# Ssellu/vslam-pose-estimation-framework

Hardware: AMD Instinct MI355X
Metric: stereo frames/sec on KITTI-00 at 1/2/4/8 MI355X; ATE vs reference (higher is better)
Workload: dtype u8

## Files before the change

vslam_pose_estimation_framework_amd/csrc/kernels_image.h:

```cpp
#pragma once
#include <hip/hip_runtime.h>
#include "dev_types.h"
#include "../../include/vslam_brief_pattern.h"
#include "../../include/vslam_orb_pattern.h"
#include "brief_footprint.h"

__constant__ int8_t c_brief[256][4] = VSLAM_BRIEF_PATTERN_INIT;
constexpr int8_t k_brief_builtin[256][4] = VSLAM_BRIEF_PATTERN_INIT;
constexpr BriefFootprint k_brief_builtin_fp = brief_footprint(k_brief_builtin);
__constant__ BriefFootprint c_brief_fp = k_brief_builtin_fp;
__constant__ int8_t c_orb[256][4] = VSLAM_ORB_PATTERN_INIT;

__device__ __forceinline__ size_t ix_side(const DevCfg& c, int s, int d) { return (size_t)s * 2 + d; }
__device__ __forceinline__ uint16_t* box_of(const DevCfg& c, const DevBuf& b, int s, int d) {
  return b.box + ix_side(c, s, d) * (size_t)c.c.rows * c.bstride;
}
__device__ __forceinline__ uint8_t* score_of(const DevCfg& c, const DevBuf& b, int s, int d) {
  return b.score8 + ix_side(c, s, d) * (size_t)c.c.rows * c.bstride;
}
__device__ __forceinline__ unsigned long long* mask_of(const DevCfg& c, const DevBuf& b, int s, int d) {
  return b.mask + ix_side(c, s, d) * (size_t)c.c.rows * c.TX;
}
__device__ __forceinline__ int16_t* kpxy_of(const DevCfg& c, const DevBuf& b, int s, int d) {
  return b.kp_xy + ix_side(c, s, d) * (size_t)c.NMAX * 2;
}
__device__ __forceinline__ uint8_t* kpscore_of(const DevCfg& c, const DevBuf& b, int s, int d) {
  return b.kp_score + ix_side(c, s, d) * (size_t)c.NMAX;
}
__device__ __forceinline__ uint8_t* desc_of(const DevCfg& c, const DevBuf& b, int s, int d) {
  return b.desc + ix_side(c, s, d) * (size_t)c.NMAX * 32;
}
__device__ __forceinline__ int32_t* rowcell_of(const DevCfg& c, const DevBuf& b, int s, int d) {
  return b.rowcell + ix_side(c, s, d) * (size_t)c.c.rows * (c.CW + 1);
}
__device__ __forceinline__ uint8_t* used_of(const DevCfg& c, const DevBuf& b, int s, int d) {
  return b.used + ix_side(c, s, d) * (size_t)c.NMAX;
}
__device__ __forceinline__ int32_t* kill_of(const DevCfg& c, const DevBuf& b, int s, int d) {
  return b.kill + ix_side(c, s, d) * (size_t)c.NMAX;
}

__device__ __forceinline__ int block_exclusive_scan(int v, int* sh, int* total) {
  const int lane = threadIdx.x & 63, w = threadIdx.x >> 6, nw = blockDim.x >> 6;
  int inc = v;
#pragma unroll
  for (int o = 1; o < 64; o <<= 1) {
    const int t = __shfl_up(inc, o, 64);
    if (lane >= o) inc += t;
  }
  __syncthreads();
  if (lane == 63) sh[w] = inc;
  __syncthreads();
  if (threadIdx.x == 0) {
    int acc = 0;
    for (int i = 0; i < nw; ++i) { const int t = sh[i]; sh[i] = acc; acc += t; }
    sh[16] = acc;
  }
  __syncthreads();
  *total = sh[16];
  return sh[w] + inc - v;
}

__device__ __forceinline__ void xcd_tile(int* tx, int* ty, int* tz, int mono = 0, int rot = 0) {
  const int gx = gridDim.x, gy = gridDim.y;
  const int tps = mono ? gx * gy : gx * gy * 2;
  const int ns = mono ? gridDim.z : gridDim.z >> 1;
  int lin = blockIdx.x + gx * (blockIdx.y + gy * blockIdx.z);
  const int per = (ns >> 3) * tps;
  if (lin < (per << 3)) { const int x = (lin + rot) & 7, j = lin >> 3, q = j / tps; lin = (x + 8 * q) * tps + (j - q * tps); }
  *tx = lin % gx;
  const int r = lin / gx;
  *ty = r % gy;
  *tz = r / gy;
}

__device__ __forceinline__ int region_threshold(const DevCfg& c, const int32_t* thr, int x, int y) {
  for (int r = 0; r < c.n_regions; ++r) {
    const DevRegion& R = c.regions[r];
    if (x >= R.x + 3 && x < R.x + R.w - 3 && y >= R.y + 3 && y < R.y + R.h - 3) return thr[r];
  }
  return -1;
}

typedef short s16x2 __attribute__((ext_vector_type(2)));
__device__ __forceinline__ s16x2 pk_min(s16x2 a, s16x2 b) { return __builtin_elementwise_min(a, b); }
__device__ __forceinline__ s16x2 pk_max(s16x2 a, s16x2 b) { return __builtin_elementwise_max(a, b); }

__device__ __forceinline__ void fast_pair_scores(const uint8_t (*t)[80], int ly0, int lx0, int ly1, int lx1, int thr0, int thr1,
                                                 int* s0, int* s1) {
  const int dx[16] = {0, 1, 2, 3, 3, 3, 2, 1, 0, -1, -2, -3, -3, -3, -2, -1};
  const int dy[16] = {3, 3, 2, 1, 0, -1, -2, -3, -3, -3, -2, -1, 0, 1, 2, 3};
  const s16x2 v = {(short)t[ly0][lx0], (short)t[ly1][lx1]};
  s16x2 d[16];
#pragma unroll
  for (int k = 0; k < 16; ++k) {
    const s16x2 p = {(short)t[ly0 + dy[k]][lx0 + dx[k]], (short)t[ly1 + dy[k]][lx1 + dx[k]]};
    d[k] = v - p;
  }
  s16x2 mn2[16], mx2[16], mn4[16], mx4[16];
#pragma unroll
  for (int k = 0; k < 16; ++k) { mn2[k] = pk_min(d[k], d[(k + 1) & 15]); mx2[k] = pk_max(d[k], d[(k + 1) & 15]); }
#pragma unroll
  for (int k = 0; k < 16; ++k) { mn4[k] = pk_min(mn2[k], mn2[(k + 2) & 15]); mx4[k] = pk_max(mx2[k], mx2[(k + 2) & 15]); }
  s16x2 A = {-1000, -1000}, Bm = {1000, 1000};
#pragma unroll
  for (int k = 0; k < 16; ++k) {
    A = pk_max(A, pk_min(pk_min(mn4[k], mn4[(k + 4) & 15]), d[(k + 8) & 15]));
    Bm = pk_min(Bm, pk_max(pk_max(mx4[k], mx4[(k + 4) & 15]), d[(k + 8) & 15]));
  }
  const int a0 = A.x, b0 = -Bm.x, a1 = A.y, b1 = -Bm.y;
  *s0 = (thr0 >= 0 && (a0 > thr0 || b0 > thr0)) ? max(thr0, max(a0, b0)) - 1 : 0;
  *s1 = (thr1 >= 0 && (a1 > thr1 || b1 > thr1)) ? max(thr1, max(a1, b1)) - 1 : 0;
}

#define VS_FB_QCAP ((VS_TILE_H + 2) * 66)
#define VS_FB_HS_BYTES ((VS_TILE_H + 8) * VS_TILE_W * 2)
#define VS_FB_DYN_LDS (((VS_FB_QCAP + 256) * 2) > VS_FB_HS_BYTES ? ((VS_FB_QCAP + 256) * 2) : VS_FB_HS_BYTES)
__global__ __launch_bounds__(256, 8) void k_fast_box(const DevCfg c, const DevBuf b) {
  extern __shared__ __align__(16) unsigned char fb_dyn[];
  __shared__ __align__(16) uint8_t tile[VS_TILE_H + 8][80];
  __shared__ __align__(4) uint8_t sc[VS_TILE_H + 2][68];
  __shared__ int32_t s_thr[VSLAM_MAX_REGIONS];
  constexpr int QCAP = VS_FB_QCAP;
  uint16_t* queue = reinterpret_cast<uint16_t*>(fb_dyn);
  uint16_t (*hs)[VS_TILE_W] = reinterpret_cast<uint16_t (*)[VS_TILE_W]>(fb_dyn);
  __shared__ unsigned long long lmask[VS_TILE_H];
  __shared__ int qn;
  int tx, ty, tz;
  xcd_tile(&tx, &ty, &tz, c.mono, b.xcd_rot);
  const int s = b.s0 + (c.mono ? tz : (tz >> 1)), side = c.mono ? 0 : (tz & 1);
  if (!vs_active(b, s)) return;
  const int x0 = tx * VS_TILE_W, y0 = ty * VS_TILE_H;
  const int rows = c.c.rows, cols = c.c.cols;
  const uint8_t* img = b.img[side] + (size_t)s * b.img_stream_stride;
  const int stride = b.img_row_stride;
  const int tid = threadIdx.x, lane = tid & 63, w = tid >> 6;
  if (tid < c.n_regions) s_thr[tid] = min(max(b.st[s].thr[tid], 0), 255);
  if (tid == 0) qn = 0;
  if (tid < VS_TILE_H) lmask[tid] = 0ull;
  for (int i = tid; i < (VS_TILE_H + 2) * 17; i += 256) reinterpret_cast<uint32_t*>(&sc[0][0])[i] = 0u;
  const bool aligned = ((stride & 3) == 0) && ((reinterpret_cast<uintptr_t>(img) & 3) == 0);
  constexpr int NST = ((VS_TILE_H + 8) * 18 + 255) / 256;
  if (aligned && x0 >= 4 && x0 + 68 <= cols) {
    uint32_t v[NST];
#pragma unroll
    for (int u = 0; u < NST; ++u) {
      const int i = tid + 256 * u;
      const int r = i / 18, q = i - r * 18;
      const int gy = min(max(y0 - 4 + r, 0), rows - 1);
      v[u] = 0;
      if (i < (VS_TILE_H + 8) * 18) v[u] = __builtin_nontemporal_load(reinterpret_cast<const uint32_t*>(img + (size_t)gy * stride + (x0 - 4 + 4 * q)));
    }
#pragma unroll
    for (int u = 0; u < NST; ++u) {
      const int i = tid + 256 * u;
      const int r = i / 18, q = i - r * 18;
      if (i < (VS_TILE_H + 8) * 18) *reinterpret_cast<uint32_t*>(&tile[r][4 * q]) = v[u];
    }
  } else {
    for (int i = tid; i < (VS_TILE_H + 8) * 18; i += 256) {
      const int r = i / 18, q = i - r * 18;
      const int gy = min(max(y0 - 4 + r, 0), rows - 1), gx0 = x0 - 4 + 4 * q;
      uint32_t v = 0;
#pragma unroll
      for (int k = 0; k < 4; ++k) v |= (uint32_t)img[(size_t)gy * stride + min(max(gx0 + k, 0), cols - 1)] << (8 * k);
      *reinterpret_cast<uint32_t*>(&tile[r][4 * q]) = v;
    }
  }
  __syncthreads();
  int uni_thr = -2, vx0 = 0, vx1 = 0, vy0 = 0, vy1 = 0;
  bool uni_full = false;
  {
    int hits = 0;
    for (int r = 0; r < c.n_regions; ++r) {
      const DevRegion& R = c.regions[r];
      const int ax0 = max(R.x + 3, x0 - 1), ax1 = min(R.x + R.w - 3, x0 + 65), ay0 = max(R.y + 3, y0 - 1), ay1 = min(R.y + R.h - 3, y0 + VS_TILE_H + 1);
      if (ax0 < ax1 && ay0 < ay1) {
        if (hits == 0) { uni_thr = s_thr[r]; vx0 = ax0 - (x0 - 1); vx1 = ax1 - (x0 - 1); vy0 = ay0 - (y0 - 1); vy1 = ay1 - (y0 - 1); }
        ++hits;
      }
    }
    if (hits != 1) uni_thr = -2;
    uni_full = uni_thr != -2 && vx0 == 0 && vx1 == 66 && vy0 == 0 && vy1 == VS_TILE_H + 2;
  }
  auto pretest = [&](int r, int cc, bool valid = true) {
    const int thr = !valid ? -1 : (uni_full ? uni_thr : region_threshold(c, s_thr, x0 - 1 + cc, y0 - 1 + r));
    bool cand = false;
    if (thr >= 0) {
      const int ly = r + 3, lx = cc + 3;
      const int v = tile[ly][lx];
      const int d0 = v - tile[ly + 3][lx], d4 = v - tile[ly][lx + 3], d8 = v - tile[ly - 3][lx], d12 = v - tile[ly][lx - 3];
      const int dk = min(max(d0, d8), max(d4, d12));
      const int br = max(min(d0, d8), min(d4, d12));
      cand = dk > thr || br < -thr;
    }
    const unsigned long long m = __ballot(cand);
    if (m) {
      int base = 0;
      if (lane == 0) base = atomicAdd(&qn, __popcll(m));
      base = __builtin_amdgcn_readfirstlane(base);
      if (cand) queue[base + __builtin_amdgcn_mbcnt_hi((uint32_t)(m >> 32), __builtin_amdgcn_mbcnt_lo((uint32_t)m, 0u))] = (uint16_t)((r << 8) | cc);
    }
  };
  if (uni_thr != -2) {
    const s16x2 thr2 = {(short)uni_thr, (short)uni_thr};
    constexpr bool RING = (VS_TILE_H % 16) == 0;
    constexpr int RBASE = RING ? 1 : 0, RCOUNT = RING ? VS_TILE_H : VS_TILE_H + 2;
#pragma unroll 1
    for (int pass = 0; pass < (RCOUNT + 15) / 16; ++pass) {
      if (pass * 16 + w * 4 >= RCOUNT) continue;
      const int r = RBASE + pass * 16 + (tid >> 4), q = (tid & 15) + 1;
      uint32_t ng0 = 0, ng1 = 0;
      if (r < RBASE + RCOUNT) {
        const uint32_t* rowp = reinterpret_cast<const uint32_t*>(&tile[r + 3][0]);
        const uint32_t C = rowp[q], C0 = rowp[q - 1], C2 = rowp[q + 1];
        const uint32_t N = reinterpret_cast<const uint32_t*>(&tile[r][0])[q], S = reinterpret_cast<const uint32_t*>(&tile[r + 6][0])[q];
#pragma unroll
        for (int half = 0; half < 2; ++half) {
          const uint32_t sel = half ? 0x0c030c02u : 0x0c010c00u;
          const uint32_t vv = __builtin_amdgcn_perm(0u, C, sel), nn = __builtin_amdgcn_perm(0u, N, sel), ss = __builtin_amdgcn_perm(0u, S, sel);
          const uint32_t ee = __builtin_amdgcn_perm(C2, C, half ? 0x0c060c05u : 0x0c040c03u);
          const uint32_t ww = __builtin_amdgcn_perm(C, C0, half ? 0x0c040c03u : 0x0c020c01u);
          const s16x2 v = __builtin_bit_cast(s16x2, vv), n = __builtin_bit_cast(s16x2, nn), s_ = __builtin_bit_cast(s16x2, ss);
          const s16x2 e = __builtin_bit_cast(s16x2, ee), w_ = __builtin_bit_cast(s16x2, ww);
          const s16x2 lo = pk_max(pk_min(n, s_), pk_min(e, w_)), hi = pk_min(pk_max(n, s_), pk_max(e, w_));
          const uint32_t neg = __builtin_bit_cast(uint32_t, (s16x2)(lo - (v - thr2))) | __builtin_bit_cast(uint32_t, (s16x2)((v + thr2) - hi));
          if (half) ng1 = neg; else ng0 = neg;
        }
      }
      bool p0 = (short)(ng0 & 0xffffu) < 0, p1 = (int)ng0 < 0, p2 = (short)(ng1 & 0xffffu) < 0, p3 = (int)ng1 < 0;
      if (!uni_full) {
        const bool rok = r >= vy0 && r < vy1;
        const int c0 = 4 * q - 3;
        p0 = p0 && rok && c0 >= vx0 && c0 < vx1;         p1 = p1 && rok && c0 + 1 >= vx0 && c0 + 1 < vx1;
        p2 = p2 && rok && c0 + 2 >= vx0 && c0 + 2 < vx1; p3 = p3 && rok && c0 + 3 >= vx0 && c0 + 3 < vx1;
      }
      const unsigned long long m0 = __ballot(p0), m1 = __ballot(p1), m2 = __ballot(p2), m3 = __ballot(p3);
      const int n0 = __popcll(m0), n1 = __popcll(m1), n2 = __popcll(m2), n3 = __popcll(m3);
      if (n0 + n1 + n2 + n3) {
        int base = 0;
        if (lane == 0) base = atomicAdd(&qn, n0 + n1 + n2 + n3);
        base = __builtin_amdgcn_readfirstlane(base);
        const int ent = (r << 8) | (4 * q - 3);
        auto below = [&](unsigned long long m) { return (int)__builtin_amdgcn_mbcnt_hi((uint32_t)(m >> 32), __builtin_amdgcn_mbcnt_lo((uint32_t)m, 0u)); };
        const int trash = QCAP + tid;
        queue[p0 ? base + below(m0) : trash] = (uint16_t)ent;
        queue[p1 ? base + n0 + below(m1) : trash] = (uint16_t)(ent + 1);
        queue[p2 ? base + n0 + n1 + below(m2) : trash] = (uint16_t)(ent + 2);
        queue[p3 ? base + n0 + n1 + n2 + below(m3) : trash] = (uint16_t)(ent + 3);
      }
    }
    if (RING) {
      constexpr int NRING = 2 * 66 + 2 * VS_TILE_H;
      for (int i0 = 0; i0 < NRING; i0 += 256) {
        const int i = i0 + tid;
        int r = 0, cc = 0;
        if (i < 66) { r = 0; cc = i; }
        else if (i < 132) { r = VS_TILE_H + 1; cc = i - 66; }
        else { const int k = i - 132; r = 1 + (k >> 1); cc = (k & 1) ? 65 : 0; }
        pretest(r, cc, i < NRING);
      }
    } else {
      if (tid >= 64 && tid < 64 + (VS_TILE_H + 2) * 2) { const int i = tid - 64; pretest(i >> 1, (i & 1) ? 65 : 0); }
    }
  } else {
    for (int r = w; r < VS_TILE_H + 2; r += 4) pretest(r, lane);
    if (tid < (VS_TILE_H + 2) * 2) pretest(tid >> 1, 64 + (tid & 1));
    static_assert((VS_TILE_H + 2) * 2 <= 256, "one pass over the halo columns");
  }
  __syncthreads();
  {
    const int nq = qn;
    for (int q = tid; 2 * q < nq; q += 256) {
      const int e0 = queue[2 * q], e1 = (2 * q + 1 < nq) ? queue[2 * q + 1] : e0;
      const int r0 = e0 >> 8, c0 = e0 & 255, r1 = e1 >> 8, c1 = e1 & 255;
      int sv0, sv1;
      const int t0 = uni_thr != -2 ? uni_thr : region_threshold(c, s_thr, x0 - 1 + c0, y0 - 1 + r0);
      const int t1 = uni_thr != -2 ? uni_thr : region_threshold(c, s_thr, x0 - 1 + c1, y0 - 1 + r1);
      fast_pair_scores(tile, r0 + 3, c0 + 3, r1 + 3, c1 + 3, t0, t1, &sv0, &sv1);
      sc[r0][c0] = (uint8_t)sv0;
      if (2 * q + 1 < nq) sc[r1][c1] = (uint8_t)sv1;
    }
  }
  __syncthreads();
  unsigned long long* mask = mask_of(c, b, s, side);
  uint8_t* score8 = score_of(c, b, s, side);
  uint16_t* box = box_of(c, b, s, side);
  {
    const int nq = qn;
    for (int q = tid; q < nq; q += 256) {
      const int e0 = queue[q];
      const int r = e0 >> 8, cc = e0 & 255;
      if (r < 1 || r > VS_TILE_H || cc < 1 || cc > 64) continue;
      const int v = sc[r][cc];
      if (v == 0) continue;
      const bool keep = v > sc[r - 1][cc - 1] && v > sc[r - 1][cc] && v > sc[r - 1][cc + 1] && v > sc[r][cc - 1] &&
                        v > sc[r][cc + 1] && v > sc[r + 1][cc - 1] && v > sc[r + 1][cc] && v > sc[r + 1][cc + 1];
      if (keep) {
        atomicOr(&lmask[r - 1], 1ull << (cc - 1));
        const int gy = y0 + r - 1;
        if (gy < rows) score8[(size_t)gy * c.bstride + (x0 + cc - 1)] = (uint8_t)v;
      }
    }
  }
  __syncthreads();
  const bool want_box = c.c.descriptor_type == VSLAM_DESCRIPTOR_BRIEF;
  if (want_box)
  for (int i = tid; i < (VS_TILE_H + 8) * 16; i += 256) {
    const int r = i >> 4, q = i & 15;
    const uint32_t* p = reinterpret_cast<const uint32_t*>(&tile[r][4 * q]);
    const uint32_t w0 = p[0], w1 = p[1], w2 = p[2];
    const uint32_t s0 = __builtin_amdgcn_sad_u8(w0, 0u, __builtin_amdgcn_sad_u8(w1, 0u, w2 & 255u));
    const uint32_t s1 = s0 - (w0 & 255u) + ((w2 >> 8) & 255u);
    const uint32_t s2 = s1 - ((w0 >> 8) & 255u) + ((w2 >> 16) & 255u);
    const uint32_t s3 = s2 - ((w0 >> 16) & 255u) + (w2 >> 24);
    *reinterpret_cast<uint2*>(&hs[r][4 * q]) = make_uint2(s0 | (s1 << 16), s2 | (s3 << 16));
  }
  __syncthreads();
  if (want_box) {
    constexpr int RW = VS_TILE_H / 8;
    const int half = lane >> 5, px = 2 * (lane & 31);
    const int rbase = (w * 2 + half) * RW;
    typedef unsigned short u16x2 __attribute__((ext_vector_type(2)));
    u16x2 acc = {0, 0};
#pragma unroll
    for (int k = 0; k < 9; ++k) acc += *reinterpret_cast<const u16x2*>(&hs[rbase + k][px]);
#pragma unroll
    for (int j = 0; j < RW; ++j) {
      const int r = rbase + j, gy = y0 + r;
      if (gy < rows && x0 + px < c.bstride) __builtin_nontemporal_store(__builtin_bit_cast(uint32_t, acc), reinterpret_cast<uint32_t*>(box + (size_t)gy * c.bstride + x0 + px));
      if (j < RW - 1) acc += *reinterpret_cast<const u16x2*>(&hs[r + 9][px]) - *reinterpret_cast<const u16x2*>(&hs[r][px]);
    }
  }
  __syncthreads();
  if (tid < VS_TILE_H && y0 + tid < rows) mask[(size_t)(y0 + tid) * c.TX + tx] = lmask[tid];
}

__device__ __forceinline__ unsigned long long col_mask(int lo, int hi, int wx0) {
  int a = max(lo - wx0, 0), e = min(hi - wx0, 64);
  if (e <= a) return 0ull;
  const unsigned long long hi_m = (e >= 64) ? ~0ull : ((1ull << e) - 1ull);
  return hi_m & ~((1ull << a) - 1ull);
}

#ifndef VS_EMIT_WPT
#define VS_EMIT_WPT 4
#endif
__global__ __launch_bounds__(512, VS_EMIT_WPT > 8 ? 2 : 4) void k_emit(const DevCfg c, const DevBuf b, int border, int run_controller) {
  __shared__ int sh_wave[8], sh_total;
  __shared__ int sh_cnt[VSLAM_MAX_REGIONS];
  __shared__ int sh_last;
  const int s = b.s0 + xcd_local_stream(blockIdx.x, gridDim.x, (b.xcd_rot + blockIdx.y * gridDim.x) & 7), tid = threadIdx.x;
  if (!vs_active(b, s)) return;
  const int rows = c.c.rows, cols = c.c.cols, TX = c.TX, CW = c.CW;
  StreamState& st = b.st[s];
  if (tid < VSLAM_MAX_REGIONS) sh_cnt[tid] = 0;
  __syncthreads();
  const int nwords = rows * TX;
  const int side = blockIdx.y, lane = tid & 63, w = tid >> 6;
  {
    const unsigned long long* mask = mask_of(c, b, s, side);
    const uint8_t* score8 = score_of(c, b, s, side);
    int16_t* kxy = kpxy_of(c, b, s, side);
    uint8_t* ksc = kpscore_of(c, b, s, side);
    int32_t* rowcell = rowcell_of(c, b, s, side);
    uint8_t* used = used_of(c, b, s, side);
    auto filtered = [&](unsigned long long m, int row, int t) -> unsigned long long {
      const bool row_ok = row >= border && row < rows - border;
      return row_ok ? (m & col_mask(border, cols - border, t * 64)) : 0ull;
    };
    int done = 0;
    const int q64 = 64 / TX, r64 = 64 - q64 * TX;
    for (int p0 = 0; p0 < nwords; p0 += 512 * VS_EMIT_WPT) {
      const int wbase = p0 + w * 64 * VS_EMIT_WPT + lane;
      const int row_b = wbase / TX, t_b = wbase - row_b * TX;
      unsigned long long mw[VS_EMIT_WPT];
#pragma unroll
      for (int j = 0; j < VS_EMIT_WPT; ++j) mw[j] = (wbase + 64 * j < nwords) ? mask[wbase + 64 * j] : 0ull;
      for (int r = 0; r < c.n_regions; ++r) {
        const DevRegion& R = c.regions[r];
        int n = 0, row = row_b, t = t_b;
#pragma unroll
        for (int j = 0; j < VS_EMIT_WPT; ++j) {
          if (row >= R.y + 3 && row < R.y + R.h - 3) n += __popcll(mw[j] & col_mask(R.x + 3, R.x + R.w - 3, t * 64));
          t += r64; row += q64; if (t >= TX) { t -= TX; ++row; }
        }
#pragma unroll
        for (int o = 32; o > 0; o >>= 1) n += __shfl_xor(n, o, 64);
        if (lane == 0 && n) atomicAdd(&sh_cnt[r], n);
      }
      int ex[VS_EMIT_WPT];
      int carry = 0;
      int row = row_b, t = t_b;
#pragma unroll
      for (int j = 0; j < VS_EMIT_WPT; ++j) {
        const int wd = wbase + 64 * j;
        mw[j] = wd < nwords ? filtered(mw[j], row, t) : 0ull;
        t += r64; row += q64; if (t >= TX) { t -= TX; ++row; }
        const int cnt = __popcll(mw[j]);
        int inc = cnt;
#pragma unroll
        for (int o = 1; o < 64; o <<= 1) { const int up = __shfl_up(inc, o, 64); if (lane >= o) inc += up; }
        ex[j] = carry + inc - cnt;
        carry += __shfl(inc, 63, 64);
      }
      __syncthreads();
      if (lane == 0) sh_wave[w] = carry;
      __syncthreads();
      if (tid == 0) { int acc = 0; for (int i = 0; i < 8; ++i) { const int v = sh_wave[i]; sh_wave[i] = acc; acc += v; } sh_total = acc; }
      __syncthreads();
      const int wave_off = done + sh_wave[w];
      row = row_b; t = t_b;
#pragma unroll
      for (int j = 0; j < VS_EMIT_WPT; ++j) {
        const int wd = wbase + 64 * j;
        if (wd < nwords) {
          unsigned long long f = mw[j];
          int off = wave_off + ex[j];
          int32_t* rc = rowcell + (size_t)row * (CW + 1) + t * 4;
          rc[0] = min(off, c.NMAX);
          rc[1] = min(off + __popcll(f & 0xFFFFull), c.NMAX);
          rc[2] = min(off + __popcll(f & 0xFFFFFFFFull), c.NMAX);
          rc[3] = min(off + __popcll(f & 0xFFFFFFFFFFFFull), c.NMAX);
          if (t == TX - 1) rc[4] = min(off + __popcll(f), c.NMAX);
          while (f) {
            const int bit = __ffsll((long long)f) - 1;
            f &= f - 1;
            if (off < c.NMAX) {
              *reinterpret_cast<int32_t*>(kxy + 2 * off) = (t * 64 + bit) | (row << 16);
              used[off] = 0;
            }
            ++off;
          }
        }
        t += r64; row += q64; if (t >= TX) { t -= TX; ++row; }
      }
      done += sh_total;
    }
    const int total = done;
    if (total > c.NMAX) { if (tid == 0) atomicOr(&st.error_flags, 1); }
    if (tid == 0) b.n_kp[s * 2 + side] = min(total, c.NMAX);
    __syncthreads();
    const int nk = min(total, c.NMAX);
    for (int i0 = tid; i0 < nk; i0 += 4 * 512) {
      int px[4];
      uint8_t v[4];
#pragma unroll
      for (int u = 0; u < 4; ++u) {
        const int i = i0 + 512 * u;
        px[u] = (i < nk) ? *reinterpret_cast<const int32_t*>(kxy + 2 * i) : 0;
      }
#pragma unroll
      for (int u = 0; u < 4; ++u) v[u] = (i0 + 512 * u < nk) ? score8[(size_t)(px[u] >> 16) * c.bstride + (px[u] & 0xFFFF)] : 0;
#pragma unroll
      for (int u = 0; u < 4; ++u) if (i0 + 512 * u < nk) ksc[i0 + 512 * u] = v[u];
    }
    __syncthreads();
  }
  if (tid == 0) {
    for (int r = 0; r < c.n_regions; ++r) b.iinfo[s].raw_count[side][r] = sh_cnt[r];
    __threadfence();
    const int last_ticket = (int)gridDim.y - 1;
    const int ticket = atomicAdd(&b.iinfo[s].ticket, 1);
    sh_last = ticket == last_ticket;
    if (ticket == last_ticket) { __threadfence(); b.iinfo[s].ticket = 0; }
  }
  __syncthreads();
  if (tid == 0 && sh_last) {
    const int (*cnt)[VSLAM_MAX_REGIONS] = b.iinfo[s].raw_count;
    if (run_controller) {
      const double tol = c.c.target_number_of_keypoints_tolerance, maxchg = c.c.detector_threshold_maximum_change;
      const double tmin = c.c.detector_threshold_minimum, tmax = c.c.detector_threshold_maximum;
      const double target = (double)c.target_per_detector;
      const int n_sides = run_controller == 2 ? 1 : 2;
      for (int r = 0; r < c.n_regions; ++r) {
        double acc = 0;
        for (int sd = 0; sd < n_sides; ++sd) {
          double t = (double)st.thr[r];
          const double delta = ((double)__hip_atomic_load(&cnt[sd][r], __ATOMIC_RELAXED, __HIP_MEMORY_SCOPE_AGENT) - target) / target;
          if (delta < -tol) {
            const double change = fmax(delta, -maxchg);
            t = t + fmin(change * t, -1.0);
            if (t < tmin) t = tmin;
          } else if (delta > tol) {
            const double change = fmin(delta, maxchg);
            t += fmax(change * t, 1.0);
            if (t > tmax) t = tmax;
          }
          acc += t;
        }
        st.thr[r] = (int)rint(acc / n_sides);
      }
    }
    for (int r = 0; r < c.n_regions; ++r) b.iinfo[s].thr_after[r] = st.thr[r];
  }
}

__device__ __forceinline__ void brief_wave(const uint16_t* box, int bstride, int x, int y, int lane, uint8_t* out32) {
#pragma unroll
  for (int j = 0; j < 4; ++j) {
    const int i = j * 64 + lane;
    const int a = box[(size_t)(y + c_brief[i][0]) * bstride + (x + c_brief[i][1])];
    const int bb = box[(size_t)(y + c_brief[i][2]) * bstride + (x + c_brief[i][3])];
    const unsigned long long m = __ballot(a < bb);
    if (lane == 0) {
      const unsigned long long wv = __builtin_bswap64(__brevll(m));
      reinterpret_cast<unsigned long long*>(out32)[j] = wv;
    }
  }
}

#ifndef VS_BT_W
#define VS_BT_W 128
#endif
#ifndef VS_BT_H
#define VS_BT_H 64
#endif
#define VS_BT_RW (VS_BT_W + 2 * VSLAM_BRIEF_PATCH_HALF)
#define VS_BT_RH (VS_BT_H + 2 * VSLAM_BRIEF_PATCH_HALF)
__global__ __launch_bounds__(256) void k_brief(const DevCfg c, const DevBuf b) {
  __shared__ __align__(16) uint16_t reg[VS_BT_RH * VS_BT_RW];
  __shared__ int row_lo[VS_BT_H], row_off[VS_BT_H + 1];
  int tx, ty, tz;
  xcd_tile(&tx, &ty, &tz, c.mono, b.xcd_rot);
  const int s = b.s0 + (c.mono ? tz : (tz >> 1)), side = c.mono ? 0 : (tz & 1);
  if (!vs_active(b, s)) return;
  const int x0 = tx * VS_BT_W, y0 = ty * VS_BT_H;
  const int rows = c.c.rows;
  const int tid = threadIdx.x, lane = tid & 63, w = tid >> 6;
  const int32_t* rowcell = rowcell_of(c, b, s, side);
  if (tid < VS_BT_H) {
    const int r = y0 + tid;
    int lo = 0, n = 0;
    if (r < rows) {
      const int c0 = min((VS_BT_W / 16) * tx, c.CW), c1 = min((VS_BT_W / 16) * (tx + 1), c.CW);
      lo = rowcell[(size_t)r * (c.CW + 1) + c0];
      n = rowcell[(size_t)r * (c.CW + 1) + c1] - lo;
    }
    row_lo[tid] = lo;
    int inc = n;
#pragma unroll
    for (int o = 1; o < VS_BT_H; o <<= 1) { const int t = __shfl_up(inc, o, 64); if (tid >= o) inc += t; }
    row_off[tid + 1] = inc;
    if (tid == 0) row_off[0] = 0;
  }
  __syncthreads();
  const int K = row_off[VS_BT_H];
  if (K == 0) return;
  const uint16_t* box = box_of(c, b, s, side);
  constexpr int CPR = VS_BT_RW / 8;
  constexpr int NLD = (VS_BT_RH * CPR + 255) / 256;
  uint4 stage[NLD];
#pragma unroll
  for (int u = 0; u < NLD; ++u) {
    const int i = tid + 256 * u;
    const int r = i / CPR, q = i - r * CPR;
    const int gy = min(max(y0 - VSLAM_BRIEF_PATCH_HALF + r, 0), rows - 1);
    const int gx = x0 - VSLAM_BRIEF_PATCH_HALF + 8 * q;
    stage[u] = make_uint4(0u, 0u, 0u, 0u);
    if (i < VS_BT_RH * CPR && gx >= 0 && gx + 8 <= c.bstride) stage[u] = *reinterpret_cast<const uint4*>(box + (size_t)gy * c.bstride + gx);
  }
  const int16_t* kxy = kpxy_of(c, b, s, side);
  auto lookup = [&](int k, int* base, int* idx) {
    *base = 0; *idx = -1;
    if (k < K) {
      int r = 0;
#pragma unroll
      for (int step = VS_BT_H / 2; step > 0; step >>= 1) if (row_off[r + step] <= k) r += step;
      const int id = row_lo[r] + (k - row_off[r]);
      *idx = id;
      *base = (r + VSLAM_BRIEF_PATCH_HALF) * VS_BT_RW + (kxy[2 * id] - x0 + VSLAM_BRIEF_PATCH_HALF);
    }
  };
  int my_base, my_idx;
  lookup(w + 4 * lane, &my_base, &my_idx);
  int off_a[4], off_b[4];
#pragma unroll
  for (int j = 0; j < 4; ++j) {
    const int i = j * 64 + lane;
    off_a[j] = c_brief[i][0] * VS_BT_RW + c_brief[i][1];
    off_b[j] = c_brief[i][2] * VS_BT_RW + c_brief[i][3];
  }
#pragma unroll
  for (int u = 0; u < NLD; ++u) {
    const int i = tid + 256 * u;
    if (i < VS_BT_RH * CPR) *reinterpret_cast<uint4*>(&reg[8 * i]) = stage[u];
  }
  __syncthreads();
  uint8_t* desc = desc_of(c, b, s, side);
  for (int k0 = 0; k0 < K; k0 += 256) {
    if (k0 > 0) lookup(k0 + w + 4 * lane, &my_base, &my_idx);
    const int n_here = (min(K - k0, 256) - w + 3) >> 2;
    for (int i = 0; i < n_here; ++i) {
      const int base = __builtin_amdgcn_readlane(my_base, i), idx = __builtin_amdgcn_readlane(my_idx, i);
      unsigned long long word = 0;
#pragma unroll
      for (int j = 0; j < 4; ++j) {
        const unsigned long long m = __ballot(reg[base + off_a[j]] < reg[base + off_b[j]]);
        if (lane == j) word = m;
      }
      if (lane < 4) reinterpret_cast<unsigned long long*>(desc + (size_t)32 * idx)[lane] = __builtin_bswap64(__brevll(word));
    }
  }
}

__global__ __launch_bounds__(256) void k_brief_at(const uint16_t* box, int bstride, int rows, int cols, int n,
                                                  const int16_t* xy, uint8_t* keep, uint8_t* desc) {
  const int lane = threadIdx.x & 63;
  const int wave = blockIdx.x * (blockDim.x >> 6) + (threadIdx.x >> 6);
  const int nwaves = gridDim.x * (blockDim.x >> 6);
  for (int i = wave; i < n; i += nwaves) {
    const int x = xy[2 * i], y = xy[2 * i + 1];
    const bool in = x >= VSLAM_BRIEF_BORDER && x < cols - VSLAM_BRIEF_BORDER && y >= VSLAM_BRIEF_BORDER && y < rows - VSLAM_BRIEF_BORDER;
    if (lane == 0) keep[i] = in ? 1 : 0;
    if (in) brief_wave(box, bstride, x, y, lane, desc + (size_t)32 * i);
    else if (lane < 4) reinterpret_cast<unsigned long long*>(desc + (size_t)32 * i)[lane] = 0ull;
  }
}

struct Gauss7 { int32_t k[4]; };
__device__ __forceinline__ int reflect101(int p, int n) { return p < 0 ? -p : (p >= n ? 2 * n - 2 - p : p); }
__device__ __forceinline__ uint8_t* blur_of(const DevCfg& c, const DevBuf& b, int s, int d) { return reinterpret_cast<uint8_t*>(box_of(c, b, s, d)); }

__device__ __forceinline__ void gauss7_tile(const uint8_t* img, int stride, int rows, int cols, int x0, int y0, const Gauss7& g, uint8_t* out, int ostride,
                                            uint8_t (*src)[72], uint16_t (*hs)[VS_TILE_W]) {
  const int tid = threadIdx.x;
  const bool in_dwords = ((stride & 3) == 0) && ((reinterpret_cast<uintptr_t>(img) & 3) == 0) && x0 >= 4 && x0 + 68 <= cols;
  if (in_dwords) {
    constexpr int NST = ((VS_TILE_H + 6) * 18 + 255) / 256;
    uint32_t v[NST];
#pragma unroll
    for (int u = 0; u < NST; ++u) {
      const int i = tid + 256 * u;
      const int r = i / 18, q = i - 18 * r;
      const int gy = reflect101(min(y0 - 3 + r, rows + 2), rows);
      v[u] = 0;
      if (i < (VS_TILE_H + 6) * 18) v[u] = *reinterpret_cast<const uint32_t*>(img + (size_t)gy * stride + (x0 - 4 + 4 * q));
    }
#pragma unroll
    for (int u = 0; u < NST; ++u) {
      const int i = tid + 256 * u;
      const int r = i / 18, q = i - 18 * r;
      if (i < (VS_TILE_H + 6) * 18) *reinterpret_cast<uint32_t*>(&src[r][4 * q]) = v[u];
    }
  } else {
    for (int i = tid; i < (VS_TILE_H + 6) * 70; i += 256) {
      const int r = i / 70, q = i - 70 * r;
      src[r][q + 1] = img[(size_t)reflect101(min(y0 - 3 + r, rows + 2), rows) * stride + reflect101(min(x0 - 3 + q, cols + 2), cols)];
    }
  }
  __syncthreads();
  const uint32_t klo = (uint32_t)g.k[3] | ((uint32_t)g.k[2] << 8) | ((uint32_t)g.k[1] << 16) | ((uint32_t)g.k[0] << 24);
  const uint32_t khi = (uint32_t)g.k[1] | ((uint32_t)g.k[2] << 8) | ((uint32_t)g.k[3] << 16);
  for (int i = tid; i < (VS_TILE_H + 6) * 16; i += 256) {
    const int r = i >> 4, t = i & 15;
    const uint32_t* p = reinterpret_cast<const uint32_t*>(&src[r][4 * t]);
    const uint32_t w0 = p[0], w1 = p[1], w2 = p[2];
    uint32_t o[4];
#pragma unroll
    for (int j = 0; j < 4; ++j) {
      const uint32_t lo = j == 3 ? w1 : __builtin_amdgcn_alignbyte(w1, w0, 1 + j), hi = j == 3 ? w2 : __builtin_amdgcn_alignbyte(w2, w1, 1 + j);
      o[j] = __builtin_amdgcn_udot4(lo, klo, __builtin_amdgcn_udot4(hi, khi, 0u, false), false);
    }
    *reinterpret_cast<uint2*>(&hs[r][4 * t]) = make_uint2(o[0] | (o[1] << 16), o[2] | (o[3] << 16));
  }
  __syncthreads();
  const bool out_dwords = ((ostride & 3) == 0) && ((reinterpret_cast<uintptr_t>(out) & 3) == 0);
  for (int i = tid; i < VS_TILE_H * 16; i += 256) {
    const int r = i >> 4, t = i & 15;
    if (y0 + r >= rows || x0 + 4 * t >= cols) continue;
    uint32_t acc[4] = {0, 0, 0, 0};
#pragma unroll
    for (int d = 0; d < 7; ++d) {
      const uint2 v = *reinterpret_cast<const uint2*>(&hs[r + d][4 * t]);
      const uint32_t kk = (uint32_t)g.k[d < 3 ? 3 - d : d - 3];
      acc[0] += kk * (v.x & 0xFFFFu); acc[1] += kk * (v.x >> 16); acc[2] += kk * (v.y & 0xFFFFu); acc[3] += kk * (v.y >> 16);
    }
    uint32_t px[4];
#pragma unroll
    for (int j = 0; j < 4; ++j) px[j] = min((acc[j] + (1u << 15)) >> 16, 255u);
    uint8_t* dst = out + (size_t)(y0 + r) * ostride + x0 + 4 * t;
    if (out_dwords && x0 + 4 * t + 4 <= (ostride > cols ? ostride : cols)) {
      *reinterpret_cast<uint32_t*>(dst) = px[0] | (px[1] << 8) | (px[2] << 16) | (px[3] << 24);
    } else {
#pragma unroll
      for (int j = 0; j < 4; ++j) if (x0 + 4 * t + j < cols) dst[j] = (uint8_t)px[j];
    }
  }
}
__global__ __launch_bounds__(256) void k_gauss7(const DevCfg c, const DevBuf b, const Gauss7 g) {
  __shared__ uint8_t src[VS_TILE_H + 6][72];
  __shared__ uint16_t hs[VS_TILE_H + 6][VS_TILE_W];
  int tx, ty, tz;
  xcd_tile(&tx, &ty, &tz, c.mono, b.xcd_rot);
  const int s = b.s0 + (c.mono ? tz : (tz >> 1)), side = c.mono ? 0 : (tz & 1);
  if (!vs_active(b, s)) return;
  gauss7_tile(b.img[side] + (size_t)s * b.img_stream_stride, b.img_row_stride, c.c.rows, c.c.cols, tx * VS_TILE_W, ty * VS_TILE_H, g,
              blur_of(c, b, s, side), c.bstride, src, hs);
}
__global__ __launch_bounds__(256) void k_gauss7_plain(const uint8_t* img, int stride, int rows, int cols, const Gauss7 g, uint8_t* out, int ostride) {
  __shared__ uint8_t src[VS_TILE_H + 6][72];
  __shared__ uint16_t hs[VS_TILE_H + 6][VS_TILE_W];
  gauss7_tile(img, stride, rows, cols, blockIdx.x * VS_TILE_W, blockIdx.y * VS_TILE_H, g, out, ostride, src, hs);
}

struct OrbTaps { int off[4][2]; };
__device__ __forceinline__ OrbTaps orb_taps(int lane, float a, float bsin, int stride) {
  OrbTaps t;
#pragma unroll
  for (int j = 0; j < 4; ++j) {
    const int i = j * 64 + lane;
#pragma unroll
    for (int h = 0; h < 2; ++h) {
      const float px = (float)c_orb[i][2 * h], py = (float)c_orb[i][2 * h + 1];
      const float xf = px * a - py * bsin, yf = px * bsin + py * a;
      t.off[j][h] = (int)rintf(yf) * stride + (int)rintf(xf);
    }
  }
  return t;
}
__device__ __forceinline__ void orb_wave(const uint8_t* centre, const OrbTaps& t, unsigned long long d[4]) {
  int v[4][2];
#pragma unroll
  for (int j = 0; j < 4; ++j) { v[j][0] = centre[t.off[j][0]]; v[j][1] = centre[t.off[j][1]]; }
#pragma unroll
  for (int j = 0; j < 4; ++j) d[j] = __ballot(v[j][0] < v[j][1]);
}
#define VS_OT_HALF 16
#define VS_OT_RW (VS_BT_W + 2 * VS_OT_HALF)
#define VS_OT_RH (VS_BT_H + 2 * VS_OT_HALF)
__global__ __launch_bounds__(256) void k_orb_describe(const DevCfg c, const DevBuf b, float a, float bsin) {
  __shared__ __align__(16) uint8_t reg[VS_OT_RH * VS_OT_RW];
  __shared__ int row_lo[VS_BT_H], row_off[VS_BT_H + 1];
  int tx, ty, tz;
  xcd_tile(&tx, &ty, &tz, c.mono, b.xcd_rot);
  const int s = b.s0 + (c.mono ? tz : (tz >> 1)), side = c.mono ? 0 : (tz & 1);
  if (!vs_active(b, s)) return;
  const int x0 = tx * VS_BT_W, y0 = ty * VS_BT_H;
  const int rows = c.c.rows;
  const int tid = threadIdx.x, lane = tid & 63, w = tid >> 6;
  const int32_t* rowcell = rowcell_of(c, b, s, side);
  if (tid < VS_BT_H) {
    const int r = y0 + tid;
    int lo = 0, n = 0;
    if (r < rows) {
      const int c0 = min((VS_BT_W / 16) * tx, c.CW), c1 = min((VS_BT_W / 16) * (tx + 1), c.CW);
      lo = rowcell[(size_t)r * (c.CW + 1) + c0];
      n = rowcell[(size_t)r * (c.CW + 1) + c1] - lo;
    }
    row_lo[tid] = lo;
    int inc = n;
#pragma unroll
    for (int o = 1; o < VS_BT_H; o <<= 1) { const int t = __shfl_up(inc, o, 64); if (tid >= o) inc += t; }
    row_off[tid + 1] = inc;
    if (tid == 0) row_off[0] = 0;
  }
  __syncthreads();
  const int K = row_off[VS_BT_H];
  if (K == 0) return;
  const uint8_t* blur = blur_of(c, b, s, side);
  constexpr int CPR = VS_OT_RW / 16;
  constexpr int NLD = (VS_OT_RH * CPR + 255) / 256;
  uint4 stage[NLD];
#pragma unroll
  for (int u = 0; u < NLD; ++u) {
    const int i = tid + 256 * u;
    const int r = i / CPR, q = i - r * CPR;
    const int gy = min(max(y0 - VS_OT_HALF + r, 0), rows - 1);
    const int gx = x0 - VS_OT_HALF + 16 * q;
    stage[u] = make_uint4(0u, 0u, 0u, 0u);
    if (i < VS_OT_RH * CPR && gx >= 0 && gx + 16 <= c.bstride) stage[u] = *reinterpret_cast<const uint4*>(blur + (size_t)gy * c.bstride + gx);
  }
  const int16_t* kxy = kpxy_of(c, b, s, side);
  auto lookup = [&](int k, int* base, int* idx) {
    *base = 0; *idx = -1;
    if (k < K) {
      int r = 0;
#pragma unroll
      for (int step = VS_BT_H / 2; step > 0; step >>= 1) if (row_off[r + step] <= k) r += step;
      const int id = row_lo[r] + (k - row_off[r]);
      *idx = id;
      *base = (r + VS_OT_HALF) * VS_OT_RW + (kxy[2 * id] - x0 + VS_OT_HALF);
    }
  };
  int my_base, my_idx;
  lookup(w + 4 * lane, &my_base, &my_idx);
  const OrbTaps t = orb_taps(lane, a, bsin, VS_OT_RW);
#pragma unroll
  for (int u = 0; u < NLD; ++u) {
    const int i = tid + 256 * u;
    if (i < VS_OT_RH * CPR) *reinterpret_cast<uint4*>(&reg[16 * i]) = stage[u];
  }
  __syncthreads();
  uint8_t* desc = desc_of(c, b, s, side);
  for (int k0 = 0; k0 < K; k0 += 256) {
    if (k0 > 0) lookup(k0 + w + 4 * lane, &my_base, &my_idx);
    const int n_here = (min(K - k0, 256) - w + 3) >> 2;
    for (int i = 0; i < n_here; ++i) {
      const int base = __builtin_amdgcn_readlane(my_base, i), idx = __builtin_amdgcn_readlane(my_idx, i);
      unsigned long long word = 0;
#pragma unroll
      for (int j = 0; j < 4; ++j) {
        const unsigned long long m = __ballot(reg[base + t.off[j][0]] < reg[base + t.off[j][1]]);
        if (lane == j) word = m;
      }
      if (lane < 4) reinterpret_cast<unsigned long long*>(desc + (size_t)32 * idx)[lane] = word;
    }
  }
}
__global__ __launch_bounds__(256) void k_orb_at(const uint8_t* blur, int stride, int rows, int cols, int n, const int16_t* xy, float a, float bsin,
                                                uint8_t* keep, uint8_t* desc) {
  const int lane = threadIdx.x & 63;
  const int wave = blockIdx.x * (blockDim.x >> 6) + (threadIdx.x >> 6), nwaves = gridDim.x * (blockDim.x >> 6);
  const OrbTaps t = orb_taps(lane, a, bsin, stride);
  for (int i = wave; i < n; i += nwaves) {
    const int x = xy[2 * i], y = xy[2 * i + 1];
    const bool in = x >= VSLAM_ORB_BORDER && x < cols - VSLAM_ORB_BORDER && y >= VSLAM_ORB_BORDER && y < rows - VSLAM_ORB_BORDER;
    if (lane == 0) keep[i] = in ? 1 : 0;
    unsigned long long d[4] = {0ull, 0ull, 0ull, 0ull};
    if (in) orb_wave(blur + (size_t)y * stride + x, t, d);
    const unsigned long long dv = lane == 0 ? d[0] : (lane == 1 ? d[1] : (lane == 2 ? d[2] : d[3]));
    if (lane < 4) reinterpret_cast<unsigned long long*>(desc + (size_t)32 * i)[lane] = dv;
  }
}

struct OrbLevels { const uint8_t* blur[16]; int32_t stride[16], rows[16], cols[16]; };
__global__ __launch_bounds__(256) void k_orb_at_levels(const OrbLevels L, int n, const int32_t* pos, const float* ab, uint8_t* keep, uint8_t* desc) {
  const int lane = threadIdx.x & 63;
  const int wave = blockIdx.x * (blockDim.x >> 6) + (threadIdx.x >> 6), nwaves = gridDim.x * (blockDim.x >> 6);
  for (int i = wave; i < n; i += nwaves) {
    const int lv = pos[3 * i + 2];
    unsigned long long d[4] = {0ull, 0ull, 0ull, 0ull};
    const bool in = lv >= 0;
    if (in) {
      const int stride = L.stride[lv];
      const OrbTaps t = orb_taps(lane, ab[2 * i], ab[2 * i + 1], stride);
      orb_wave(L.blur[lv] + (size_t)pos[3 * i + 1] * stride + pos[3 * i], t, d);
    }
    if (lane == 0) keep[i] = in ? 1 : 0;
    const unsigned long long dv = lane == 0 ? d[0] : (lane == 1 ? d[1] : (lane == 2 ? d[2] : d[3]));
    if (lane < 4) reinterpret_cast<unsigned long long*>(desc + (size_t)32 * i)[lane] = dv;
  }
}

enum { VS_KNN_HAMMING = 0, VS_KNN_L2 = 1, VS_KNN_L1 = 2, VS_KNN_SL2 = 3 };
#define VS_KNN_TILE 256
__device__ __forceinline__ void knn_merge(unsigned long long& b0, unsigned long long& b1, unsigned long long c0, unsigned long long c1) {
  const unsigned long long lo = b0 < c0 ? b0 : c0, hi = b0 < c0 ? c0 : b0, m = b1 < c1 ? b1 : c1;
  b0 = lo; b1 = hi < m ? hi : m;
}
template <int NORM>
__device__ __forceinline__ void knn2_body(int nq, const uint8_t* __restrict__ q, int nt, const uint8_t* __restrict__ t, int32_t* idx,
                                          float* dist, uint4 (*tile)[2], uint32_t* tnorm) {
  const int tid = threadIdx.x, sub = tid & 15, grp = tid >> 4;
  const int i = blockIdx.x * 16 + grp;
  const bool dotn = NORM == VS_KNN_L2 || NORM == VS_KNN_SL2;
  uint32_t qv[8];
  uint32_t qn = 0;
  {
    const uint4* qp = reinterpret_cast<const uint4*>(q + (size_t)32 * (i < nq ? i : nq - 1));
    const uint4 a = qp[0], c = qp[1];
    qv[0] = a.x; qv[1] = a.y; qv[2] = a.z; qv[3] = a.w; qv[4] = c.x; qv[5] = c.y; qv[6] = c.z; qv[7] = c.w;
    if (dotn) {
#pragma unroll
      for (int k = 0; k < 8; ++k) qn = __builtin_amdgcn_udot4(qv[k], qv[k], qn, false);
    }
  }
  unsigned long long b0 = ~0ull, b1 = ~0ull;
  uint4 n0 = make_uint4(0, 0, 0, 0), n1 = n0;
  if (tid < nt) { const uint4* tp = reinterpret_cast<const uint4*>(t + (size_t)32 * tid); n0 = tp[0]; n1 = tp[1]; }
  for (int j0 = 0; j0 < nt; j0 += VS_KNN_TILE) {
    __syncthreads();
    {
      const int sw = (tid >> 3) & 1;
      tile[tid][sw] = n0; tile[tid][sw ^ 1] = n1;
      if (dotn) {
        uint32_t tn = 0;
        tn = __builtin_amdgcn_udot4(n0.x, n0.x, tn, false); tn = __builtin_amdgcn_udot4(n0.y, n0.y, tn, false);
        tn = __builtin_amdgcn_udot4(n0.z, n0.z, tn, false); tn = __builtin_amdgcn_udot4(n0.w, n0.w, tn, false);
        tn = __builtin_amdgcn_udot4(n1.x, n1.x, tn, false); tn = __builtin_amdgcn_udot4(n1.y, n1.y, tn, false);
        tn = __builtin_amdgcn_udot4(n1.z, n1.z, tn, false); tn = __builtin_amdgcn_udot4(n1.w, n1.w, tn, false);
        tnorm[tid] = tn;
      }
    }
    const int jn = j0 + VS_KNN_TILE;
    if (jn + tid < nt) { const uint4* tp = reinterpret_cast<const uint4*>(t + (size_t)32 * (jn + tid)); n0 = tp[0]; n1 = tp[1]; }
    __syncthreads();
    const int cnt = min(VS_KNN_TILE, nt - j0);
    for (int r = sub; r < cnt; r += 16) {
      const int sw = (r >> 3) & 1;
      const uint4 a = tile[r][sw], c = tile[r][sw ^ 1];
      const uint32_t tv[8] = {a.x, a.y, a.z, a.w, c.x, c.y, c.z, c.w};
      uint32_t d = 0;
      if (NORM == VS_KNN_HAMMING) {
#pragma unroll
        for (int k = 0; k < 8; ++k) d += __popc(qv[k] ^ tv[k]);
      } else if (NORM == VS_KNN_L1) {
#pragma unroll
        for (int k = 0; k < 8; ++k) d = __builtin_amdgcn_sad_u8(qv[k], tv[k], d);
      } else {
        uint32_t dot = 0;
#pragma unroll
        for (int k = 0; k < 8; ++k) dot = __builtin_amdgcn_udot4(qv[k], tv[k], dot, false);
        d = qn + tnorm[r] - 2u * dot;
      }
      const unsigned long long key = ((unsigned long long)d << 32) | (unsigned)(j0 + r);
      if (key < b0) { b1 = b0; b0 = key; }
      else if (key < b1) { b1 = key; }
    }
  }
#pragma unroll
  for (int m = 1; m < 16; m <<= 1) {
    const unsigned long long c0 = __shfl_xor(b0, m, 64), c1 = __shfl_xor(b1, m, 64);
    knn_merge(b0, b1, c0, c1);
  }
  if (i < nq && sub == 0) {
    const bool h0 = b0 != ~0ull, h1 = b1 != ~0ull;
    idx[2 * i] = h0 ? (int32_t)(b0 & 0xFFFFFFFFull) : -1;
    idx[2 * i + 1] = h1 ? (int32_t)(b1 & 0xFFFFFFFFull) : -1;
    const float d0 = (float)(uint32_t)(b0 >> 32), d1 = (float)(uint32_t)(b1 >> 32);
    dist[2 * i] = h0 ? (NORM == VS_KNN_L2 ? sqrtf(d0) : d0) : 0.f;
    dist[2 * i + 1] = h1 ? (NORM == VS_KNN_L2 ? sqrtf(d1) : d1) : 0.f;
  }
}
__global__ __launch_bounds__(256) void k_knn2(int norm, int nq, const uint8_t* __restrict__ q, int nt,
                                              const uint8_t* __restrict__ t, int32_t* idx, float* dist) {
  __shared__ uint4 tile[VS_KNN_TILE][2];
  __shared__ uint32_t tnorm[VS_KNN_TILE];
  if (norm == VS_KNN_HAMMING) knn2_body<VS_KNN_HAMMING>(nq, q, nt, t, idx, dist, tile, tnorm);
  else if (norm == VS_KNN_L2) knn2_body<VS_KNN_L2>(nq, q, nt, t, idx, dist, tile, tnorm);
  else if (norm == VS_KNN_L1) knn2_body<VS_KNN_L1>(nq, q, nt, t, idx, dist, tile, tnorm);
  else knn2_body<VS_KNN_SL2>(nq, q, nt, t, idx, dist, tile, tnorm);
}
```

Before: 187,000.

## Rewrite FAST score as f16 packed min3/max3 over pixels; simplify candidate queue

The FAST corner score now works on raw pixel values packed into f16 (via the 0x6400 exponent trick) and takes windowed min/max with three-input min3/max3 ops. The centre pixel is subtracted once at the end instead of forming 16 differences first. The pretest loop precomputes column-validity masks and folds the row range into one bound check. It also uses an inline-asm LDS fetch-add, replaces trash-slot stores with predicated stores, drops the queue padding, and skips wholly idle waves on the ring pass. The goal is fewer VALU instructions and less LDS use. The risks are correctness of the windowed min/max reduction, and the asm waitcnt serialising the atomic.

Result: faster. 195,100 (median of 6 runs) (+4.3%).

```diff
diff --git a/vslam_pose_estimation_framework_amd/csrc/kernels_image.h b/vslam_pose_estimation_framework_amd/csrc/kernels_image.h
--- a/vslam_pose_estimation_framework_amd/csrc/kernels_image.h
+++ b/vslam_pose_estimation_framework_amd/csrc/kernels_image.h
@@ -86,42 +86,51 @@
 __device__ __forceinline__ s16x2 pk_min(s16x2 a, s16x2 b) { return __builtin_elementwise_min(a, b); }
 __device__ __forceinline__ s16x2 pk_max(s16x2 a, s16x2 b) { return __builtin_elementwise_max(a, b); }
 
+typedef _Float16 h16x2 __attribute__((ext_vector_type(2)));
+__device__ __forceinline__ h16x2 pk_min3(h16x2 a, h16x2 b, h16x2 c) { return __builtin_elementwise_minimum(__builtin_elementwise_minimum(a, b), c); }
+__device__ __forceinline__ h16x2 pk_max3(h16x2 a, h16x2 b, h16x2 c) { return __builtin_elementwise_maximum(__builtin_elementwise_maximum(a, b), c); }
+
 __device__ __forceinline__ void fast_pair_scores(const uint8_t (*t)[80], int ly0, int lx0, int ly1, int lx1, int thr0, int thr1,
                                                  int* s0, int* s1) {
   const int dx[16] = {0, 1, 2, 3, 3, 3, 2, 1, 0, -1, -2, -3, -3, -3, -2, -1};
   const int dy[16] = {3, 3, 2, 1, 0, -1, -2, -3, -3, -3, -2, -1, 0, 1, 2, 3};
-  const s16x2 v = {(short)t[ly0][lx0], (short)t[ly1][lx1]};
-  s16x2 d[16];
-#pragma unroll
-  for (int k = 0; k < 16; ++k) {
-    const s16x2 p = {(short)t[ly0 + dy[k]][lx0 + dx[k]], (short)t[ly1 + dy[k]][lx1 + dx[k]]};
-    d[k] = v - p;
-  }
-  s16x2 mn2[16], mx2[16], mn4[16], mx4[16];
-#pragma unroll
-  for (int k = 0; k < 16; ++k) { mn2[k] = pk_min(d[k], d[(k + 1) & 15]); mx2[k] = pk_max(d[k], d[(k + 1) & 15]); }
-#pragma unroll
-  for (int k = 0; k < 16; ++k) { mn4[k] = pk_min(mn2[k], mn2[(k + 2) & 15]); mx4[k] = pk_max(mx2[k], mx2[(k + 2) & 15]); }
-  s16x2 A = {-1000, -1000}, Bm = {1000, 1000};
-#pragma unroll
-  for (int k = 0; k < 16; ++k) {
-    A = pk_max(A, pk_min(pk_min(mn4[k], mn4[(k + 4) & 15]), d[(k + 8) & 15]));
-    Bm = pk_min(Bm, pk_max(pk_max(mx4[k], mx4[(k + 4) & 15]), d[(k + 8) & 15]));
-  }
-  const int a0 = A.x, b0 = -Bm.x, a1 = A.y, b1 = -Bm.y;
+  h16x2 p[16];
+#pragma unroll
+  for (int k = 0; k < 16; ++k)
+    p[k] = __builtin_bit_cast(h16x2, (uint32_t)t[ly0 + dy[k]][lx0 + dx[k]] | ((uint32_t)t[ly1 + dy[k]][lx1 + dx[k]] << 16) | 0x64006400u);
+  h16x2 mn3[16], mx3[16], amn[16], amx[16];
+#pragma unroll
+  for (int k = 0; k < 16; ++k) { mn3[k] = pk_min3(p[k], p[(k + 1) & 15], p[(k + 2) & 15]); mx3[k] = pk_max3(p[k], p[(k + 1) & 15], p[(k + 2) & 15]); }
+#pragma unroll
+  for (int k = 0; k < 16; ++k) { amn[k] = pk_min3(mn3[k], mn3[(k + 3) & 15], mn3[(k + 6) & 15]); amx[k] = pk_max3(mx3[k], mx3[(k + 3) & 15], mx3[(k + 6) & 15]); }
+  h16x2 M6[6], m6[6];
+#pragma unroll
+  for (int k = 0; k < 5; ++k) { M6[k] = pk_min3(amx[3 * k], amx[3 * k + 1], amx[3 * k + 2]); m6[k] = pk_max3(amn[3 * k], amn[3 * k + 1], amn[3 * k + 2]); }
+  M6[5] = amx[15]; m6[5] = amn[15];
+  const h16x2 M2 = pk_min3(pk_min3(M6[0], M6[1], M6[2]), pk_min3(M6[3], M6[4], M6[5]), M6[5]);
+  const h16x2 m2 = pk_max3(pk_max3(m6[0], m6[1], m6[2]), pk_max3(m6[3], m6[4], m6[5]), m6[5]);
+  const uint32_t Mb = __builtin_bit_cast(uint32_t, M2), mb = __builtin_bit_cast(uint32_t, m2);
+  const int v0 = t[ly0][lx0], v1 = t[ly1][lx1];
+  const int a0 = v0 - (int)(Mb & 0x3ffu), b0 = (int)(mb & 0x3ffu) - v0, a1 = v1 - (int)((Mb >> 16) & 0x3ffu), b1 = (int)((mb >> 16) & 0x3ffu) - v1;
   *s0 = (thr0 >= 0 && (a0 > thr0 || b0 > thr0)) ? max(thr0, max(a0, b0)) - 1 : 0;
   *s1 = (thr1 >= 0 && (a1 > thr1 || b1 > thr1)) ? max(thr1, max(a1, b1)) - 1 : 0;
 }
 
+__device__ __forceinline__ int lds_fetch_add(int* word, int v) {
+  const uint32_t addr = (uint32_t)reinterpret_cast<uintptr_t>((__attribute__((address_space(3))) int*)word);
+  int old;
+  asm volatile("ds_add_rtn_u32 %0, %1, %2\n\ts_waitcnt lgkmcnt(0)" : "=&v"(old) : "v"(addr), "v"(v) : "memory");
+  return old;
+}
+
 #define VS_FB_QCAP ((VS_TILE_H + 2) * 66)
 #define VS_FB_HS_BYTES ((VS_TILE_H + 8) * VS_TILE_W * 2)
-#define VS_FB_DYN_LDS (((VS_FB_QCAP + 256) * 2) > VS_FB_HS_BYTES ? ((VS_FB_QCAP + 256) * 2) : VS_FB_HS_BYTES)
+#define VS_FB_DYN_LDS ((VS_FB_QCAP * 2) > VS_FB_HS_BYTES ? (VS_FB_QCAP * 2) : VS_FB_HS_BYTES)
 __global__ __launch_bounds__(256, 8) void k_fast_box(const DevCfg c, const DevBuf b) {
   extern __shared__ __align__(16) unsigned char fb_dyn[];
   __shared__ __align__(16) uint8_t tile[VS_TILE_H + 8][80];
   __shared__ __align__(4) uint8_t sc[VS_TILE_H + 2][68];
   __shared__ int32_t s_thr[VSLAM_MAX_REGIONS];
-  constexpr int QCAP = VS_FB_QCAP;
   uint16_t* queue = reinterpret_cast<uint16_t*>(fb_dyn);
   uint16_t (*hs)[VS_TILE_W] = reinterpret_cast<uint16_t (*)[VS_TILE_W]>(fb_dyn);
   __shared__ unsigned long long lmask[VS_TILE_H];
@@ -197,7 +206,7 @@
     const unsigned long long m = __ballot(cand);
     if (m) {
       int base = 0;
-      if (lane == 0) base = atomicAdd(&qn, __popcll(m));
+      if (lane == 0) base = lds_fetch_add(&qn, __popcll(m));
       base = __builtin_amdgcn_readfirstlane(base);
       if (cand) queue[base + __builtin_amdgcn_mbcnt_hi((uint32_t)(m >> 32), __builtin_amdgcn_mbcnt_lo((uint32_t)m, 0u))] = (uint16_t)((r << 8) | cc);
     }
@@ -206,12 +215,19 @@
     const s16x2 thr2 = {(short)uni_thr, (short)uni_thr};
     constexpr bool RING = (VS_TILE_H % 16) == 0;
     constexpr int RBASE = RING ? 1 : 0, RCOUNT = RING ? VS_TILE_H : VS_TILE_H + 2;
+    const int rlo = max(RBASE, vy0), rhi = min(RBASE + RCOUNT, vy1);
+    uint32_t cm0 = 0x80008000u, cm1 = 0x80008000u;
+    if (!uni_full) {
+      const int c0 = 4 * ((tid & 15) + 1) - 3;
+      cm0 = (c0 >= vx0 && c0 < vx1 ? 0x8000u : 0u) | (c0 + 1 >= vx0 && c0 + 1 < vx1 ? 0x80000000u : 0u);
+      cm1 = (c0 + 2 >= vx0 && c0 + 2 < vx1 ? 0x8000u : 0u) | (c0 + 3 >= vx0 && c0 + 3 < vx1 ? 0x80000000u : 0u);
+    }
 #pragma unroll 1
     for (int pass = 0; pass < (RCOUNT + 15) / 16; ++pass) {
-      if (pass * 16 + w * 4 >= RCOUNT) continue;
+      if (RCOUNT % 16 != 0 && pass * 16 + w * 4 >= RCOUNT) continue;
       const int r = RBASE + pass * 16 + (tid >> 4), q = (tid & 15) + 1;
       uint32_t ng0 = 0, ng1 = 0;
-      if (r < RBASE + RCOUNT) {
+      if ((unsigned)(r - rlo) < (unsigned)(rhi - rlo)) {
         const uint32_t* rowp = reinterpret_cast<const uint32_t*>(&tile[r + 3][0]);
         const uint32_t C = rowp[q], C0 = rowp[q - 1], C2 = rowp[q + 1];
         const uint32_t N = reinterpret_cast<const uint32_t*>(&tile[r][0])[q], S = reinterpret_cast<const uint32_t*>(&tile[r + 6][0])[q];
@@ -225,34 +241,30 @@
           const s16x2 e = __builtin_bit_cast(s16x2, ee), w_ = __builtin_bit_cast(s16x2, ww);
           const s16x2 lo = pk_max(pk_min(n, s_), pk_min(e, w_)), hi = pk_min(pk_max(n, s_), pk_max(e, w_));
           const uint32_t neg = __builtin_bit_cast(uint32_t, (s16x2)(lo - (v - thr2))) | __builtin_bit_cast(uint32_t, (s16x2)((v + thr2) - hi));
-          if (half) ng1 = neg; else ng0 = neg;
+          if (half) ng1 = neg & cm1; else ng0 = neg & cm0;
         }
       }
-      bool p0 = (short)(ng0 & 0xffffu) < 0, p1 = (int)ng0 < 0, p2 = (short)(ng1 & 0xffffu) < 0, p3 = (int)ng1 < 0;
-      if (!uni_full) {
-        const bool rok = r >= vy0 && r < vy1;
-        const int c0 = 4 * q - 3;
-        p0 = p0 && rok && c0 >= vx0 && c0 < vx1;         p1 = p1 && rok && c0 + 1 >= vx0 && c0 + 1 < vx1;
-        p2 = p2 && rok && c0 + 2 >= vx0 && c0 + 2 < vx1; p3 = p3 && rok && c0 + 3 >= vx0 && c0 + 3 < vx1;
-      }
+      uint32_t lo0 = ng0 << 16, lo1 = ng1 << 16;
+      asm("" : "+v"(lo0), "+v"(lo1));
+      const bool p0 = (int)lo0 < 0, p1 = (int)ng0 < 0, p2 = (int)lo1 < 0, p3 = (int)ng1 < 0;
       const unsigned long long m0 = __ballot(p0), m1 = __ballot(p1), m2 = __ballot(p2), m3 = __ballot(p3);
       const int n0 = __popcll(m0), n1 = __popcll(m1), n2 = __popcll(m2), n3 = __popcll(m3);
       if (n0 + n1 + n2 + n3) {
         int base = 0;
-        if (lane == 0) base = atomicAdd(&qn, n0 + n1 + n2 + n3);
+        if (lane == 0) base = lds_fetch_add(&qn, n0 + n1 + n2 + n3);
         base = __builtin_amdgcn_readfirstlane(base);
-        const int ent = (r << 8) | (4 * q - 3);
+        const int ent = (r << 8) + (4 * q - 3);
         auto below = [&](unsigned long long m) { return (int)__builtin_amdgcn_mbcnt_hi((uint32_t)(m >> 32), __builtin_amdgcn_mbcnt_lo((uint32_t)m, 0u)); };
-        const int trash = QCAP + tid;
-        queue[p0 ? base + below(m0) : trash] = (uint16_t)ent;
-        queue[p1 ? base + n0 + below(m1) : trash] = (uint16_t)(ent + 1);
-        queue[p2 ? base + n0 + n1 + below(m2) : trash] = (uint16_t)(ent + 2);
-        queue[p3 ? base + n0 + n1 + n2 + below(m3) : trash] = (uint16_t)(ent + 3);
+        if (p0) queue[base + below(m0)] = (uint16_t)ent;
+        if (p1) queue[base + n0 + below(m1)] = (uint16_t)(ent + 1);
+        if (p2) queue[base + n0 + n1 + below(m2)] = (uint16_t)(ent + 2);
+        if (p3) queue[base + n0 + n1 + n2 + below(m3)] = (uint16_t)(ent + 3);
       }
     }
     if (RING) {
       constexpr int NRING = 2 * 66 + 2 * VS_TILE_H;
       for (int i0 = 0; i0 < NRING; i0 += 256) {
+        if (i0 + 64 * w >= NRING) continue;
         const int i = i0 + tid;
         int r = 0, cc = 0;
         if (i < 66) { r = 0; cc = i; }
```
